# entn-at/exemplars_vc

Hardware: AMD Instinct MI355X
Metric: spectral frames/sec converted (100 NMF iters, N=4096 dict) (higher is better)
Workload: dtype f64

## Files before the change

exemplars_vc_amd/csrc/evc_fused_all.hip:

```cpp
#include "evc_fused_common.h"

namespace evc {

constexpr int AW = 4;
constexpr int AKT = 8;
constexpr int ATILES = AW * AKT;
constexpr int ATHREADS = 2 * AW * 64;
constexpr unsigned ALL_POLL_LIMIT = 1u << 17;
constexpr int ALL_STAGGER_PER_ITER = 11000;
constexpr int ALL_EXCH_PRIO = 3;
typedef unsigned all_u32x4 __attribute__((ext_vector_type(4)));
typedef long long all_i64x2 __attribute__((ext_vector_type(2)));

__device__ __forceinline__ bool all_polls_out(unsigned& polls, const int* coop_abort) {
    return ++polls > ALL_POLL_LIMIT ||
           ((polls & 63) == 0 && __hip_atomic_load(coop_abort, __ATOMIC_RELAXED, __HIP_MEMORY_SCOPE_AGENT) != 0);
}

constexpr long ALL_LDS_BUDGET = 160 * 1024 - 256;
__host__ __device__ constexpr int all_dict_row(int e) { return 4 * (((e >> 2) & 1) * 2 + (e >> 3)) + (e & 3); }
template <int MSTEPS, int C, bool KL>
struct AllShape {
    static constexpr int MT = MSTEPS > 4 ? 2 : 1;
    static constexpr int E = MT * 4 * 64;
    static constexpr int NE = MSTEPS * 64;
    static constexpr int RSTR = NE < 256 ? 256 : NE;
    static constexpr int STG = C > 0 ? 1 : (C == 0 ? NE : NE + ALL_MAX_MEMBERS - 1);
    static constexpr long REST = 8L * 2 * (AW * RSTR + 2 * E + (KL ? E : 1) + STG) + 3 * 4;
    static constexpr long dict_bytes(int pr) { return 8L * ATILES * 16 * pr; }
    static constexpr int PR_ALL = 4 * MSTEPS + 2;
    static constexpr int PR = KL ? 0
                              : REST + dict_bytes(PR_ALL) <= ALL_LDS_BUDGET       ? PR_ALL
                              : REST + dict_bytes(PR_ALL - 4) <= ALL_LDS_BUDGET   ? PR_ALL - 4
                                                                                  : 0;
    static constexpr bool LDS_DICT = C != 1 && PR > 0 && PR - 1 >= 4 * MSTEPS - 3;
};

#ifdef EVC_ALL_TIMING
#define EVC_STAMP(i)                                                                                             \
    do {                                                                                                         \
        if (a.dbg && tt0 == g - half && lane == 0 && w == 0)                                                     \
            a.dbg[(((long)blockIdx.x * 2 + half) * (2 * a.iters + 1) + step) * 4 + (i)] = __builtin_amdgcn_s_memtime(); \
    } while (0)
#else
#define EVC_STAMP(i)
#endif

template <int MSTEPS, int C, bool KL>
__global__ __launch_bounds__(ATHREADS, 2) void k_fused_all(FusedArgs a) {
    using S = AllShape<MSTEPS, C, KL>;
    constexpr int MT = S::MT;
    constexpr int E = S::E;
    constexpr int NE = S::NE;
    constexpr int RSTR = S::RSTR;
    constexpr int MSP = (MSTEPS + 1) & ~1;
    constexpr int PR = S::PR;
    constexpr int TPD = 16 * PR;
    __shared__ __attribute__((aligned(16))) double s_red[2][AW * RSTR];
    __shared__ __attribute__((aligned(16))) double s_v[2][E];
    __shared__ __attribute__((aligned(16))) double s_x[2][E];
    __shared__ __attribute__((aligned(16))) double s_r[2][KL ? E : 1];
    __shared__ double s_stage[2][S::STG];
    __shared__ double s_dict[S::LDS_DICT ? ATILES * TPD : 1];
    __shared__ unsigned s_hb[2];
    __shared__ int s_fail;
    const int tid = threadIdx.x, lane = tid & 63;
    const int w8 = __builtin_amdgcn_readfirstlane(tid >> 6);
    const int half = w8 >> 2, w = w8 & 3, th = tid & (AW * 64 - 1);
    const int CR = C > 0 ? C : a.coop_c;
    const int member = blockIdx.x % CR;
    const int g = 2 * (blockIdx.x / CR) + half;
    double* const red = s_red[half];
    double* const vL = s_v[half];
    double* const xL = s_x[half];
    double* const rL = s_r[half];
    double* const stage = s_stage[half];
    unsigned hb = 0;
    const double* __restrict__ A1p = a.A1p;
    const double* __restrict__ A2p = a.A2p;
    f64x2* __restrict__ Hp = a.Hp;
    const int NT = a.NT;
    const long tile0 = (long)member * ATILES + w;
    const unsigned ul = (unsigned)lane;
    long sw = 0;

    const __amdgpu_buffer_rsrc_t r1 = __builtin_amdgcn_make_buffer_rsrc(const_cast<double*>(A1p), 0, NT * (MSP * 512), 0x00020000);
    const __amdgpu_buffer_rsrc_t r2 = __builtin_amdgcn_make_buffer_rsrc(const_cast<double*>(A2p), 0, NT * (MT * 2048), 0x00020000);
    const __amdgpu_buffer_rsrc_t rx = __builtin_amdgcn_make_buffer_rsrc(a.coop_buf, 0, C > 1 ? 2 * a.groups * (C * 4096) : 0, 0x00020000);
#ifdef EVC_ALL_NOFRAG
    bool nofrag_go = false;
#endif
    const unsigned ul16 = ul * 16u;
    constexpr int BL = 16 * ((MSTEPS - 1) >> 2) + 4 * ((MSTEPS - 1) & 3);
    const int rowA = w * AKT * TPD + all_dict_row(4 * (lane & 3) + ((lane & 15) >> 2)) * PR;
    const int rowB = w * AKT * TPD + all_dict_row(4 * (lane >> 4)) * PR;
    const double* const dA = s_dict + rowA + (lane >> 4);
    const double* const dAL = s_dict + rowA + min(lane >> 4, a.M - BL);
    const double* const dB = s_dict + rowB + (lane & 15);
    const double* const dBL = s_dict + rowB + min(lane & 15, a.M - 16 * (MT - 1));
#define LDS_NO_PAIR() asm volatile("" ::: "memory")
    auto load_a1 = [&](double (&a1)[MSTEPS], int k, auto lds) {
        if constexpr (decltype(lds)::value) {
#pragma unroll
            for (int s = 0; s < MSTEPS; ++s) {
                a1[s] = (s == MSTEPS - 1 ? dAL : dA)[k * TPD + 16 * (s >> 2) + 4 * (s & 3)];
                LDS_NO_PAIR();
            }
            return;
        }
#ifdef EVC_ALL_NOFRAG
        if (nofrag_go) return;
#endif
        const int so = (int)(tile0 + sw + AW * k) * (MSP * 512);
#pragma unroll
        for (int s = 0; s < MSTEPS; s += 2) {
            if (s + 1 < MSTEPS) {
                const f64x2 v = __builtin_bit_cast(f64x2, __builtin_amdgcn_raw_buffer_load_b128(r1, ul16 + (s >> 1) * 1024, so, 0));
                a1[s] = v[0];
                a1[s + 1] = v[1];
            } else {
                a1[s] = __builtin_bit_cast(double, __builtin_amdgcn_raw_buffer_load_b64(r1, ul16 + (s >> 1) * 1024, so, 0));
            }
        }
    };
    auto load_a2 = [&](double (&a2)[MT][4], int k, auto lds) {
        if constexpr (decltype(lds)::value) {
#pragma unroll
            for (int u = 0; u < MT; ++u)
#pragma unroll
                for (int r = 0; r < 4; ++r) {
                    a2[u][r] = (u == MT - 1 ? dBL : dB)[k * TPD + r * PR + 16 * u];
                    LDS_NO_PAIR();
                }
            return;
        }
#ifdef EVC_ALL_NOFRAG
        if (nofrag_go) return;
#endif
        const int so = (int)(tile0 + sw + AW * k) * (MT * 2048);
#pragma unroll
        for (int u = 0; u < MT; ++u)
#pragma unroll
            for (int r = 0; r < 4; r += 2) {
                const f64x2 v = __builtin_bit_cast(f64x2, __builtin_amdgcn_raw_buffer_load_b128(r2, ul16 + (u * 2 + (r >> 1)) * 1024, so, 0));
                a2[u][r] = v[0];
                a2[u][r + 1] = v[1];
            }
    };

    const int mode = a.eps_mode;
    const double eps = a.eps;
    const double d0 = a.l1 + (mode == EVC_EPS_ADD ? a.eps : 0.0);
    const f64x4 dinit = {d0, d0, d0, d0};
    const unsigned lo = fast_lo(mode, eps);
    unsigned seq = 0;
    int rs_es = 1, rs_len = 0, rs_pub0 = 0, rs_pub1 = 0, rs_src0 = -1, rs_src1 = -1, rs_src2 = -1;
    if (C < 0) {
        rs_es = (NE + CR - 1) / CR;
        rs_len = NE - member * rs_es;
        rs_len = rs_len < 0 ? 0 : (rs_len > rs_es ? rs_es : rs_len);
        const int e0 = th, e1 = th + AW * 64;
        const int j0 = e0 / rs_es, j1 = (e1 < NE ? e1 : e0) / rs_es;
        rs_pub0 = (j0 * CR + member) * rs_es + (e0 - j0 * rs_es);
        rs_pub1 = (j1 * CR + member) * rs_es + ((e1 < NE ? e1 : e0) - j1 * rs_es);
        auto src = [&](int idx) {
            if (idx >= CR * rs_es) return -1;
            const int el = idx % rs_es;
            return el < rs_len ? member * CR * rs_es + idx : -1;
        };
        rs_src0 = src(th);
        rs_src1 = src(th + AW * 64);
        rs_src2 = src(th + 2 * AW * 64);
    }
    if (tid == 0) s_fail = 0;
    if (tid < 2) s_hb[tid] = 0;

    if (a.stagger_cycles > 0 && ((blockIdx.x / CR) & 1)) {
        const long long t0 = __builtin_amdgcn_s_memtime();
        while (__builtin_amdgcn_s_memtime() - t0 < a.stagger_cycles) __builtin_amdgcn_s_sleep(32);
    }

    auto run = [&](auto lds) __attribute__((always_inline)) {
    for (long tt0 = g - half; tt0 < a.TT; tt0 += a.groups) {
        const long tt = tt0 + half;
        bool valid;
        {
            const long t = 16 * tt + (lane & 15);
            int u = -1;
            if (tt < a.TT && t < a.T_) u = a.frame_utt[t];
            const bool live = tt < a.TT && ((t >= a.T_) || ((u >= 0) && (a.active[u] != 0)));
            const int v0 = __syncthreads_and(half == 0 ? live : true);
            const int v1 = __syncthreads_and(half == 1 ? live : true);
            valid = (half ? v1 : v0) != 0;
        }
        HTile h[AKT];
        f64x4 p[AKT];
        double a1[MSTEPS], a2[MT][4];
        if (valid && a.first && a.init_const) {
            auto h0_of = [&](int fr) {
                const long t = 16 * tt + fr;
                const int u = t < a.T_ ? a.frame_utt[t] : -1;
                return u >= 0 ? a.h0[u] : 0.0;
            };
            for (int e = th; e < E; e += AW * 64) {
                const int s = e >> 6, l = e & 63;
                const bool in = s < MSTEPS;
                xL[e] = in ? a.Xp[(tt * MSTEPS + s) * 64 + l] : 0.0;
                vL[e] = in ? a.rsum[bin_of(s, l >> 4)] * h0_of(l & 15) : 0.0;
                if (KL) rL[e] = xL[e] / (vL[e] < a.eps ? a.eps : vL[e]);
            }
            const double hv = h0_of(lane & 15);
#pragma unroll
            for (int k = 0; k < AKT; ++k) {
                const long n0 = 16 * (tile0 + AW * k) + 4 * (lane >> 4);
#pragma unroll
                for (int r = 0; r < 4; ++r) h[k][r] = n0 + r < a.N ? hv : 0.0;
            }
        } else if (valid) {
            for (int e = th; e < E; e += AW * 64) {
                const int s = e >> 6, l = e & 63;
                const bool in = s < MSTEPS;
                xL[e] = in ? a.Xp[(tt * MSTEPS + s) * 64 + l] : 0.0;
                vL[e] = in ? a.Vp[(tt * 8 + s) * 64 + l] : 0.0;
                if (KL) rL[e] = xL[e] / (vL[e] < a.eps ? a.eps : vL[e]);
            }
#pragma unroll
            for (int k = 0; k < AKT; ++k) {
                const f64x2* t = Hp + (tt * NT + tile0 + AW * k) * 128;
                const f64x2 h01 = t[ul], h23 = t[ul + 64];
                h[k][0] = h01[0]; h[k][1] = h01[1]; h[k][2] = h23[0]; h[k][3] = h23[1];
            }
        }
        __syncthreads();
        if (valid && !KL) {
            double x[MSTEPS];
#pragma unroll
            for (int s = 0; s < MSTEPS; ++s) x[s] = xL[s * 64 + lane];
            load_a1(a1, 0, lds);
#pragma unroll
            for (int k = 0; k < AKT; ++k) {
                f64x4 acc = {0, 0, 0, 0};
#pragma unroll
                for (int s = 0; s < MSTEPS; ++s) acc = Mma<double>::mma(a1[s], x[s], acc);
                if (!decltype(lds)::value || k + 1 < AKT) load_a1(a1, (k + 1) % AKT, lds);
                p[k] = acc;
            }
        }

        if (valid && KL) load_a1(a1, 0, lds);
        for (int step = 0; step <= 2 * a.iters; ++step) {
#ifdef EVC_ALL_NOFRAG
            nofrag_go = step > 2;
#endif
            const bool mine = C == 1 ? (step & 1) == 0 : (step & 1) == half;
            EVC_STAMP(0);
            if (valid && mine && step < 2 * a.iters) {
                asm volatile("" : "+s"(sw));
                double v[MSTEPS];
#pragma unroll
                for (int s = 0; s < MSTEPS; ++s) v[s] = KL ? rL[s * 64 + lane] : vL[s * 64 + lane];
                if constexpr (decltype(lds)::value) load_a1(a1, 0, lds);
                f64x4 vn[MT];
#pragma unroll
                for (int u = 0; u < MT; ++u) vn[u] = f64x4{0, 0, 0, 0};
#pragma unroll
                for (int k = 0; k < AKT; ++k) {
                    __builtin_amdgcn_sched_barrier(0);
                    load_a2(a2, k, lds);
                    f64x4 d = KL ? f64x4{0, 0, 0, 0} : dinit;
#pragma unroll
                    for (int s = 0; s < MSTEPS; ++s) d = Mma<double>::mma(a1[s], v[s], d);
                    if (!decltype(lds)::value || k + 1 < AKT)
                        load_a1(a1, (k + 1) % AKT, lds);
                    __builtin_amdgcn_sched_barrier(0);
                    if (KL) {
#pragma unroll
                        for (int r = 0; r < 4; ++r) h[k][r] *= d[r];
                    } else {
                        mu_tile_guarded(h[k], p[k], d, mode, eps, lo);
                    }
#pragma unroll
                    for (int u = 0; u < MT; ++u)
#pragma unroll
                        for (int r = 0; r < 4; ++r) vn[u] = Mma<double>::mma(a2[u][r], h[k][r], vn[u]);
                }
#pragma unroll
                for (int u = 0; u < MT; ++u)
#pragma unroll
                    for (int r = 0; r < 4; ++r)
                        if (u * 4 + r < MSTEPS) red[w * RSTR + (u * 4 + r) * 64 + lane] = vn[u][r];
            } else if (C > 1 && valid && !mine && step > 0) {
                __builtin_amdgcn_s_setprio(ALL_EXCH_PRIO);
                const bool act = th < NE / 2;
                const int ep = act ? 2 * th : 0;
                f64x2 sm = {0.0, 0.0};
                if (w * 64 < NE / 2) {
                    f64x2 pv[AW];
#pragma unroll
                    for (int ww = 0; ww < AW; ++ww) pv[ww] = *reinterpret_cast<const f64x2*>(red + ww * RSTR + ep);
                    static_assert(AW == 4, "the four partials are named one by one");
                    asm volatile("" : "+v"(pv[0]), "+v"(pv[1]), "+v"(pv[2]), "+v"(pv[3]));
#pragma unroll
                    for (int ww = 0; ww < AW; ++ww) sm += pv[ww];
                    const long long tag = (seq >> 1) & 1;
                    const long long m0 = (__double_as_longlong(sm[0]) & ~1LL) | tag;
                    const long long m1 = (__double_as_longlong(sm[1]) & ~1LL) | tag;
                    const int xo = __builtin_amdgcn_readfirstlane((int)(((seq & 1) * (unsigned)a.groups + (unsigned)g) * (unsigned)(C * 4096)));
                    if (act)
                        __builtin_amdgcn_raw_buffer_store_b128(__builtin_bit_cast(all_u32x4, all_i64x2{m0, m1}), rx, ep * 8,
                                                               xo + member * 4096, 16);
                    bool ok = true;
                    unsigned polls = 0;
                    {
                        const long long* sp = reinterpret_cast<const long long*>(a.coop_buf) +
                                              ((size_t)(seq & 1) * a.groups + g) * (size_t)(C * 512) +
                                              (lane < C ? lane : 0) * 512 + (NE - 1);
                        for (;;) {
                            const long long b = __hip_atomic_load(sp, __ATOMIC_RELAXED, __HIP_MEMORY_SCOPE_AGENT);
                            const bool ready = lane >= C || lane == member || (b & 1) == tag;
                            if (__all(ready)) break;
                            if (all_polls_out(polls, a.coop_abort)) {
                                ok = false;
                                break;
                            }
                            __builtin_amdgcn_s_sleep(2);
                        }
                    }
                    all_i64x2 b[C > 0 ? C : 1] = {};
                    polls = 0;
                    while (__builtin_expect(ok && act, 1)) {
                        asm volatile("" ::: "memory");
#pragma unroll
                        for (int m = 0; m < C; ++m)
                            if (m != member)
                                b[m] = __builtin_bit_cast(all_i64x2, __builtin_amdgcn_raw_buffer_load_b128(rx, ep * 8, xo + m * 4096, 16));
                        long long bad = 0;
#pragma unroll
                        for (int m = 0; m < C; ++m) {
                            b[m] = (m == member) ? all_i64x2{m0, m1} : b[m];
                            bad |= (b[m][0] ^ tag) | (b[m][1] ^ tag);
                        }
                        if ((bad & 1) == 0) break;
                        if (all_polls_out(polls, a.coop_abort)) {
                            ok = false;
                            break;
                        }
                        __builtin_amdgcn_s_sleep(2);
                    }
                    f64x2 v2 = {0.0, 0.0};
#pragma unroll
                    for (int m = 0; m < C; ++m) {
                        v2[0] += __longlong_as_double(b[m][0] & ~1LL);
                        v2[1] += __longlong_as_double(b[m][1] & ~1LL);
                    }
                    if (!ok) s_fail = 1;
                    if (act) {
                        *reinterpret_cast<f64x2*>(vL + ep) = v2;
                        if (KL) {
                            const f64x2 x2 = *reinterpret_cast<const f64x2*>(xL + ep);
                            *reinterpret_cast<f64x2*>(rL + ep) =
                                f64x2{x2[0] / (v2[0] < a.eps ? a.eps : v2[0]), x2[1] / (v2[1] < a.eps ? a.eps : v2[1])};
                        }
                    }
                }
                ++seq;
                __builtin_amdgcn_s_setprio(0);
            } else if (valid && !mine && step > 0) {
                const int e0 = C <= 0 ? th % NE : th, e1 = th + AW * 64;
                const bool has1 = e1 < NE;
                __builtin_amdgcn_s_setprio(ALL_EXCH_PRIO);
                double s0 = 0.0, s1 = 0.0;
#pragma unroll
                for (int ww = 0; ww < AW; ++ww) {
                    s0 += red[ww * RSTR + e0];
                    s1 += red[ww * RSTR + (has1 ? e1 : e0)];
                }
                if (C < 0) {
                    long long* xb1 = reinterpret_cast<long long*>(a.coop_buf) +
                                     ((size_t)(seq & 1) * a.groups + g) * (size_t)CR * ALL_RS_STRIDE;
                    long long* xb2 = reinterpret_cast<long long*>(a.coop_buf) + ALL_SLICE_OFFSET +
                                     ((size_t)(seq & 1) * a.groups + g) * 512;
                    const long long tag = (seq >> 1) & 1;
                    __hip_atomic_store(xb1 + rs_pub0, (__double_as_longlong(s0) & ~1LL) | tag, __ATOMIC_RELAXED,
                                       __HIP_MEMORY_SCOPE_AGENT);
                    if (has1)
                        __hip_atomic_store(xb1 + rs_pub1, (__double_as_longlong(s1) & ~1LL) | tag, __ATOMIC_RELAXED,
                                           __HIP_MEMORY_SCOPE_AGENT);
                    bool ok = true;
                    auto fetch3 = [&](const long long* p0, const long long* p1, const long long* p2, long long& b0,
                                      long long& b1, long long& b2) {
                        unsigned polls = 0;
                        for (;;) {
                            b0 = __hip_atomic_load(p0, __ATOMIC_RELAXED, __HIP_MEMORY_SCOPE_AGENT);
                            b1 = __hip_atomic_load(p1, __ATOMIC_RELAXED, __HIP_MEMORY_SCOPE_AGENT);
                            b2 = __hip_atomic_load(p2, __ATOMIC_RELAXED, __HIP_MEMORY_SCOPE_AGENT);
                            if (__all(!ok || (((b0 ^ tag) | (b1 ^ tag) | (b2 ^ tag)) & 1) == 0)) break;
                            if (all_polls_out(polls, a.coop_abort))
                                ok = false;
                            __builtin_amdgcn_s_sleep(1);
                        }
                    };
                    {
                        long long b0, b1, b2;
                        const long long* own = xb1 + rs_pub0;
                        fetch3(rs_src0 >= 0 ? xb1 + rs_src0 : own, rs_src1 >= 0 ? xb1 + rs_src1 : own,
                               rs_src2 >= 0 ? xb1 + rs_src2 : own, b0, b1, b2);
                        if (rs_src0 >= 0) stage[th] = __longlong_as_double(b0 & ~1LL);
                        if (rs_src1 >= 0) stage[th + AW * 64] = __longlong_as_double(b1 & ~1LL);
                        if (rs_src2 >= 0) stage[th + 2 * AW * 64] = __longlong_as_double(b2 & ~1LL);
                        hb += AW;
                        if (lane == 0)
                            __hip_atomic_fetch_add(&s_hb[half], 1u, __ATOMIC_RELEASE, __HIP_MEMORY_SCOPE_WORKGROUP);
                        while ((int)(__hip_atomic_load(&s_hb[half], __ATOMIC_ACQUIRE, __HIP_MEMORY_SCOPE_WORKGROUP) - hb) < 0)
                            __builtin_amdgcn_s_sleep(1);
                        const int q = th & 3;
                        for (int el = th >> 2; el < rs_len; el += AW * 16) {
                            double v = 0.0;
                            for (int m = q; m < CR; m += 4) v += stage[m * rs_es + el];
                            v += __shfl_xor(v, 1, 64);
                            v += __shfl_xor(v, 2, 64);
                            if (q == 0)
                                __hip_atomic_store(xb2 + member * rs_es + el, (__double_as_longlong(v) & ~1LL) | tag,
                                                   __ATOMIC_RELAXED, __HIP_MEMORY_SCOPE_AGENT);
                        }
                    }
                    long long g0, g1, g2;
                    fetch3(xb2 + e0, xb2 + (has1 ? e1 : e0), xb2 + e0, g0, g1, g2);
                    s0 = __longlong_as_double(g0 & ~1LL);
                    s1 = __longlong_as_double(g1 & ~1LL);
                    ++seq;
                    if (!ok) s_fail = 1;
                } else if (C == 0) {
                    const int ES = NE / CR;
                    long long* xb1 = reinterpret_cast<long long*>(a.coop_buf) +
                                     ((size_t)(seq & 1) * a.groups + g) * (size_t)CR * 512;
                    long long* xb2 = reinterpret_cast<long long*>(a.coop_buf) + ALL_SLICE_OFFSET +
                                     ((size_t)(seq & 1) * a.groups + g) * 512;
                    const long long tag = (seq >> 1) & 1;
                    {
                        const int j0 = e0 / ES, j1 = (has1 ? e1 : e0) / ES;
                        __hip_atomic_store(xb1 + ((size_t)j0 * CR + member) * ES + (e0 - j0 * ES),
                                           (__double_as_longlong(s0) & ~1LL) | tag, __ATOMIC_RELAXED,
                                           __HIP_MEMORY_SCOPE_AGENT);
                        if (has1)
                            __hip_atomic_store(xb1 + ((size_t)j1 * CR + member) * ES + (e1 - j1 * ES),
                                               (__double_as_longlong(s1) & ~1LL) | tag, __ATOMIC_RELAXED,
                                               __HIP_MEMORY_SCOPE_AGENT);
                    }
                    bool ok = true;
                    auto fetch2 = [&](const long long* p0, const long long* p1, long long& b0, long long& b1) {
                        unsigned polls = 0;
                        for (;;) {
                            b0 = __hip_atomic_load(p0, __ATOMIC_RELAXED, __HIP_MEMORY_SCOPE_AGENT);
                            b1 = __hip_atomic_load(p1, __ATOMIC_RELAXED, __HIP_MEMORY_SCOPE_AGENT);
                            if (__all(!ok || (((b0 ^ tag) | (b1 ^ tag)) & 1) == 0)) break;
                            if (all_polls_out(polls, a.coop_abort))
                                ok = false;
                            __builtin_amdgcn_s_sleep(1);
                        }
                    };
                    {
                        long long b0, b1;
                        const long long* mine_ = xb1 + (size_t)member * NE;
                        fetch2(mine_ + e0, mine_ + (has1 ? e1 : e0), b0, b1);
                        stage[e0] = __longlong_as_double(b0 & ~1LL);
                        if (has1) stage[e1] = __longlong_as_double(b1 & ~1LL);
                        hb += AW;
                        if (lane == 0)
                            __hip_atomic_fetch_add(&s_hb[half], 1u, __ATOMIC_RELEASE, __HIP_MEMORY_SCOPE_WORKGROUP);
                        while ((int)(__hip_atomic_load(&s_hb[half], __ATOMIC_ACQUIRE, __HIP_MEMORY_SCOPE_WORKGROUP) - hb) < 0)
                            __builtin_amdgcn_s_sleep(1);
                        if (th < 4 * ES) {
                            const int el = th >> 2, q = th & 3, per = CR >> 2;
                            double v = 0.0;
                            for (int i = 0; i < per; ++i) v += stage[(q * per + i) * ES + el];
                            v += __shfl_xor(v, 1, 64);
                            v += __shfl_xor(v, 2, 64);
                            if (q == 0)
                                __hip_atomic_store(xb2 + member * ES + el, (__double_as_longlong(v) & ~1LL) | tag,
                                                   __ATOMIC_RELAXED, __HIP_MEMORY_SCOPE_AGENT);
                        }
                    }
                    long long g0, g1;
                    fetch2(xb2 + e0, xb2 + (has1 ? e1 : e0), g0, g1);
                    s0 = __longlong_as_double(g0 & ~1LL);
                    s1 = __longlong_as_double(g1 & ~1LL);
                    ++seq;
                    if (!ok) s_fail = 1;
                }
                vL[e0] = s0;
                if (has1) vL[e1] = s1;
                if (KL) {
                    rL[e0] = xL[e0] / (s0 < a.eps ? a.eps : s0);
                    if (has1) rL[e1] = xL[e1] / (s1 < a.eps ? a.eps : s1);
                }
                __builtin_amdgcn_s_setprio(0);
            }
            EVC_STAMP(1);
            __syncthreads();
            EVC_STAMP(2);
            if (C != 1 && s_fail) {
                if (tid == 0) __hip_atomic_store(a.coop_abort, 1, __ATOMIC_RELAXED, __HIP_MEMORY_SCOPE_AGENT);
                return;
            }
        }

        auto y_tail = [&](auto ut) __attribute__((always_inline)) {
            constexpr int UT = decltype(ut)::value;
            f64x4 yn[UT];
#pragma unroll
            for (int u = 0; u < UT; ++u) yn[u] = f64x4{0, 0, 0, 0};
            if (valid) {
                const __amdgpu_buffer_rsrc_t rb = __builtin_amdgcn_make_buffer_rsrc(const_cast<double*>(a.Yb2p), 0, NT * (UT * 2048), 0x00020000);
#pragma unroll
                for (int k = 0; k < AKT; ++k) {
                    const int so = (int)(tile0 + AW * k) * (UT * 2048);
                    double b2[UT][4];
#pragma unroll
                    for (int u = 0; u < UT; ++u)
#pragma unroll
                        for (int r = 0; r < 4; r += 2) {
                            const f64x2 v = __builtin_bit_cast(f64x2, __builtin_amdgcn_raw_buffer_load_b128(rb, ul16 + (u * 2 + (r >> 1)) * 1024, so, 0));
                            b2[u][r] = v[0];
                            b2[u][r + 1] = v[1];
                        }
#pragma unroll
                    for (int u = 0; u < UT; ++u)
#pragma unroll
                        for (int r = 0; r < 4; ++r) yn[u] = Mma<double>::mma(b2[u][r], h[k][r], yn[u]);
                }
            }
#pragma unroll
            for (int u = 0; u < UT; ++u) {
                if (valid) {
#pragma unroll
                    for (int r = 0; r < 4; ++r) red[w * RSTR + r * 64 + lane] = yn[u][r];
                }
                __syncthreads();
                if (valid) {
                    double y = 0.0;
#pragma unroll
                    for (int ww = 0; ww < AW; ++ww) y += red[ww * RSTR + th];
                    a.Yslab[member * a.y_stride + (tt * 8 + 4 * u) * 64 + th] = y;
                }
                __syncthreads();
            }
        };
        if (a.Yslab) {
            if (MT > 1 && a.y_mt == 1) y_tail(std::integral_constant<int, 1>{});
            else y_tail(std::integral_constant<int, MT>{});
        }
        if (valid) {
            if (!a.skip_hp) {
#pragma unroll
                for (int k = 0; k < AKT; ++k) {
                    f64x2* t = Hp + (tt * NT + tile0 + AW * k) * 128;
                    t[ul] = f64x2{h[k][0], h[k][1]};
                    t[ul + 64] = f64x2{h[k][2], h[k][3]};
                }
            }
            if (a.Hx) {
                const long t = 16 * tt + (lane & 15);
                if (t < a.T_ && a.hx_wide) {
#pragma unroll
                    for (int k = 0; k < AKT; ++k) {
                        const long n0 = 16 * (tile0 + AW * k) + 4 * (lane >> 4);
                        double* const row = a.Hx + t * a.ldhx + n0;
#pragma unroll
                        for (int r = 0; r < 4; r += 2) {
                            if (n0 + r + 1 < a.N) *reinterpret_cast<f64x2*>(row + r) = f64x2{h[k][r], h[k][r + 1]};
                            else if (n0 + r < a.N) row[r] = h[k][r];
                        }
                    }
                } else if (t < a.T_) {
#pragma unroll
                    for (int k = 0; k < AKT; ++k) {
                        const long n0 = 16 * (tile0 + AW * k) + 4 * (lane >> 4);
#pragma unroll
                        for (int r = 0; r < 4; ++r)
                            if (n0 + r < a.N) {
                                if (a.hx_frame_major) a.Hx[t * a.ldhx + n0 + r] = h[k][r];
                                else a.Hx[(n0 + r) * a.ldhx + t] = h[k][r];
                            }
                    }
                }
            }
            if (member == 0) {
                for (int e = th; e < NE; e += AW * 64) a.Vp[(tt * 8 + (e >> 6)) * 64 + (e & 63)] = vL[e];
                if (a.write_err && w == 0) {
                    double e = 0.0;
#pragma unroll
                    for (int s = 0; s < MSTEPS; ++s) {
                        const double x = xL[s * 64 + lane], vv = vL[s * 64 + lane];
                        e += KL ? kl_terms(x, vv, a.eps) : (x - vv) * (x - vv);
                    }
                    e += __shfl_xor(e, 16, 64);
                    e += __shfl_xor(e, 32, 64);
                    const long t = 16 * tt + lane;
                    if (lane < 16 && t < a.T_) a.err2[t] = e;
                }
            }
        }
        __syncthreads();
    }
    };

    if constexpr (S::LDS_DICT) {
        if (a.M > 0 && a.M < PR) {
            for (int x = tid; x < ATILES * TPD; x += ATHREADS) {
                const int slot = x / TPD, e = all_dict_row((x / PR) % 16), b = x % PR;
                const long j = (long)member * ATILES + slot / AKT + AW * (slot % AKT);
                const int q = e >> 2, r = e & 3;
                s_dict[x] = b < a.M ? A2p[((j * MT + (b >> 4)) * 2 + (r >> 1)) * 128 + (16 * q + (b & 15)) * 2 + (r & 1)] : 0.0;
            }
            __syncthreads();
            run(std::true_type{});
            return;
        }
    }
    run(std::false_type{});
}

template <int MSTEPS, int C, bool KL>
static hipError_t launch_all(FusedArgs a, int n_cus, hipStream_t s) {
    int occ = 0;
    hipError_t e = hipOccupancyMaxActiveBlocksPerMultiprocessor(&occ, k_fused_all<MSTEPS, C, KL>, ATHREADS, 0);
    if (e != hipSuccess) return e;
    if (occ < 1) return hipErrorInvalidValue;
    long resident = n_cus;
    if (2 * resident > ALL_MAX_WGS) resident = ALL_MAX_WGS / 2;
    const int cr = C > 0 ? C : a.coop_c;
    if (C == 0 && (cr < 8 || cr > 64 || (cr & (cr - 1)))) return hipErrorInvalidValue;
    if (C < 0 && (cr < 2 || cr > ALL_MAX_MEMBERS)) return hipErrorInvalidValue;
    int pairs = (int)(resident / cr);
    const int want = (a.TT + 1) / 2;
    if (pairs > want) pairs = want;
    if (pairs < 1) return hipErrorInvalidValue;
    a.groups = 2 * pairs;
    a.stagger_cycles = (a.iters > 0 && a.iters <= 25 && a.TT >= 4L * a.groups && pairs >= 2) ? (long long)a.iters * ALL_STAGGER_PER_ITER : 0;
    if (C > 1 && (reinterpret_cast<uintptr_t>(a.coop_buf) & 15)) return hipErrorInvalidValue;
    if (C != 1) {
        e = hipMemsetAsync(a.coop_buf, 0xFF, sizeof(double) * 2 * (size_t)a.groups * cr * (C < 0 ? ALL_RS_STRIDE : 512), s);
        if (e != hipSuccess) return e;
    }
    if (C <= 0) {
        if (2L * a.groups * 512 > ALL_SLICE_ELEMS) return hipErrorInvalidValue;
        e = hipMemsetAsync(a.coop_buf + ALL_SLICE_OFFSET, 0xFF, sizeof(double) * 2 * (size_t)a.groups * 512, s);
        if (e != hipSuccess) return e;
    }
    hipLaunchKernelGGL((k_fused_all<MSTEPS, C, KL>), dim3((unsigned)(pairs * cr)), dim3(ATHREADS), 0, s, a);
    return hipGetLastError();
}

template <int MSTEPS, bool KL>
static hipError_t pick_c(const FusedArgs& a, int n_cus, hipStream_t s) {
    switch (a.NT / ATILES) {
        case 1: return launch_all<MSTEPS, 1, KL>(a, n_cus, s);
        case 2: return launch_all<MSTEPS, 2, KL>(a, n_cus, s);
        case 4: return launch_all<MSTEPS, 4, KL>(a, n_cus, s);
        case 8:
            if constexpr (AllShape<MSTEPS, 8, KL>::LDS_DICT)
                if (a.M > 0 && a.M < AllShape<MSTEPS, 8, KL>::PR) return launch_all<MSTEPS, 8, KL>(a, n_cus, s);
            return launch_all<MSTEPS, 0, KL>(a, n_cus, s);
        case 16:
        case 32:
        case 64: return launch_all<MSTEPS, 0, KL>(a, n_cus, s);
        default: return launch_all<MSTEPS, -1, KL>(a, n_cus, s);
    }
}

int fused_all_members(int NT, int N, int eps_mode, int exact_div, int loss) {
    if (eps_mode == EVC_EPS_NONE || exact_div || (loss != EVC_LOSS_FROBENIUS && loss != EVC_LOSS_KL)) return 0;
    if (NT % ATILES) return 0;
    const int c = NT / ATILES;
    if (loss == EVC_LOSS_KL && c >= 2 && c < 16) return 0;
    return (c >= 1 && c <= ALL_MAX_MEMBERS) ? c : 0;
}

hipError_t fused_all_launch(int msteps, const FusedArgs& a, int n_cus, hipStream_t s) {
    if (a.NT % ATILES || !a.coop_buf || !a.coop_abort) return hipErrorInvalidValue;
    switch (msteps) {
        case 1: return a.loss == EVC_LOSS_KL ? pick_c<1, true>(a, n_cus, s) : pick_c<1, false>(a, n_cus, s);
        case 2: return a.loss == EVC_LOSS_KL ? pick_c<2, true>(a, n_cus, s) : pick_c<2, false>(a, n_cus, s);
        case 3: return a.loss == EVC_LOSS_KL ? pick_c<3, true>(a, n_cus, s) : pick_c<3, false>(a, n_cus, s);
        case 4: return a.loss == EVC_LOSS_KL ? pick_c<4, true>(a, n_cus, s) : pick_c<4, false>(a, n_cus, s);
        case 5: return a.loss == EVC_LOSS_KL ? pick_c<5, true>(a, n_cus, s) : pick_c<5, false>(a, n_cus, s);
        case 6: return a.loss == EVC_LOSS_KL ? pick_c<6, true>(a, n_cus, s) : pick_c<6, false>(a, n_cus, s);
        case 7: return a.loss == EVC_LOSS_KL ? pick_c<7, true>(a, n_cus, s) : pick_c<7, false>(a, n_cus, s);
        case 8: return a.loss == EVC_LOSS_KL ? pick_c<8, true>(a, n_cus, s) : pick_c<8, false>(a, n_cus, s);
        default: return hipErrorInvalidValue;
    }
}

}
```

Baseline: 1.130 million.

## Prefetch next-step operands before the block barrier and double-buffer fail flags

When the dictionary lives in LDS and blocks cooperate, each half now loads its next-step v/r operands and first dictionary fragment right after finishing the current step. It first meets the other waves of its half at a per-half rendezvous, so the LDS loads overlap the __syncthreads wait instead of starting after it. The shared fail flag is split into two parity slots and read one step later, so the abort check no longer depends on a value written in the same step; a final check after the loop covers both slots. This adds extra intra-half spin synchronisation and holds the operand registers across the barrier, which may raise register pressure. Timing instrumentation is also extended to stamp every tile.

New measurement: 1.140 million, median of 6. Within noise of the previous version (+0.8%).

```diff
diff --git a/exemplars_vc_amd/csrc/evc_fused_all.hip b/exemplars_vc_amd/csrc/evc_fused_all.hip
--- a/exemplars_vc_amd/csrc/evc_fused_all.hip
+++ b/exemplars_vc_amd/csrc/evc_fused_all.hip
@@ -26,7 +26,7 @@
     static constexpr int NE = MSTEPS * 64;
     static constexpr int RSTR = NE < 256 ? 256 : NE;
     static constexpr int STG = C > 0 ? 1 : (C == 0 ? NE : NE + ALL_MAX_MEMBERS - 1);
-    static constexpr long REST = 8L * 2 * (AW * RSTR + 2 * E + (KL ? E : 1) + STG) + 3 * 4;
+    static constexpr long REST = 8L * 2 * (AW * RSTR + 2 * E + (KL ? E : 1) + STG) + 4 * 4;
     static constexpr long dict_bytes(int pr) { return 8L * ATILES * 16 * pr; }
     static constexpr int PR_ALL = 4 * MSTEPS + 2;
     static constexpr int PR = KL ? 0
@@ -37,13 +37,22 @@
 };
 
 #ifdef EVC_ALL_TIMING
+#define EVC_STAMP_ROW()                                                                                          \
+    const long dbg_row = (((long)blockIdx.x * 2 + half) * ((a.TT + a.groups - 1) / a.groups) + (tt0 - (g - half)) / a.groups) * \
+                         (2 * a.iters + 1)
 #define EVC_STAMP(i)                                                                                             \
     do {                                                                                                         \
-        if (a.dbg && tt0 == g - half && lane == 0 && w == 0)                                                     \
-            a.dbg[(((long)blockIdx.x * 2 + half) * (2 * a.iters + 1) + step) * 4 + (i)] = __builtin_amdgcn_s_memtime(); \
+        if (a.dbg && lane == 0 && w == 0) a.dbg[(dbg_row + step) * 4 + (i)] = __builtin_amdgcn_s_memtime();        \
+    } while (0)
+#define EVC_STAMP_OPERANDS()                                                                                     \
+    do {                                                                                                         \
+        asm volatile("s_waitcnt lgkmcnt(0)" ::: "memory");                                                       \
+        EVC_STAMP(3);                                                                                            \
     } while (0)
 #else
+#define EVC_STAMP_ROW()
 #define EVC_STAMP(i)
+#define EVC_STAMP_OPERANDS()
 #endif
 
 template <int MSTEPS, int C, bool KL>
@@ -63,7 +72,7 @@
     __shared__ double s_stage[2][S::STG];
     __shared__ double s_dict[S::LDS_DICT ? ATILES * TPD : 1];
     __shared__ unsigned s_hb[2];
-    __shared__ int s_fail;
+    __shared__ int s_fail[2];
     const int tid = threadIdx.x, lane = tid & 63;
     const int w8 = __builtin_amdgcn_readfirstlane(tid >> 6);
     const int half = w8 >> 2, w = w8 & 3, th = tid & (AW * 64 - 1);
@@ -172,7 +181,7 @@
         rs_src1 = src(th + AW * 64);
         rs_src2 = src(th + 2 * AW * 64);
     }
-    if (tid == 0) s_fail = 0;
+    if (tid < 2) s_fail[tid] = 0;
     if (tid < 2) s_hb[tid] = 0;
 
     if (a.stagger_cycles > 0 && ((blockIdx.x / CR) & 1)) {
@@ -183,6 +192,7 @@
     auto run = [&](auto lds) __attribute__((always_inline)) {
     for (long tt0 = g - half; tt0 < a.TT; tt0 += a.groups) {
         const long tt = tt0 + half;
+        EVC_STAMP_ROW();
         bool valid;
         {
             const long t = 16 * tt + (lane & 15);
@@ -248,18 +258,37 @@
         }
 
         if (valid && KL) load_a1(a1, 0, lds);
+        double v[MSTEPS];
+        constexpr bool PRE = decltype(lds)::value && C != 1;
+        auto next_operands = [&]() __attribute__((always_inline)) {
+#pragma unroll
+            for (int s = 0; s < MSTEPS; ++s) v[s] = KL ? rL[s * 64 + lane] : vL[s * 64 + lane];
+            load_a1(a1, 0, lds);
+        };
+        auto half_rendezvous = [&]() __attribute__((always_inline)) {
+            hb += AW;
+            if (lane == 0) __hip_atomic_fetch_add(&s_hb[half], 1u, __ATOMIC_RELEASE, __HIP_MEMORY_SCOPE_WORKGROUP);
+            while ((int)(__hip_atomic_load(&s_hb[half], __ATOMIC_ACQUIRE, __HIP_MEMORY_SCOPE_WORKGROUP) - hb) < 0)
+                __builtin_amdgcn_s_sleep(1);
+        };
+        if constexpr (PRE) {
+            if (valid) next_operands();
+        }
         for (int step = 0; step <= 2 * a.iters; ++step) {
 #ifdef EVC_ALL_NOFRAG
             nofrag_go = step > 2;
 #endif
             const bool mine = C == 1 ? (step & 1) == 0 : (step & 1) == half;
             EVC_STAMP(0);
+            const int failed = C != 1 ? s_fail[(step & 1) ^ 1] : 0;
             if (valid && mine && step < 2 * a.iters) {
                 asm volatile("" : "+s"(sw));
-                double v[MSTEPS];
-#pragma unroll
-                for (int s = 0; s < MSTEPS; ++s) v[s] = KL ? rL[s * 64 + lane] : vL[s * 64 + lane];
-                if constexpr (decltype(lds)::value) load_a1(a1, 0, lds);
+                if constexpr (!PRE) {
+#pragma unroll
+                    for (int s = 0; s < MSTEPS; ++s) v[s] = KL ? rL[s * 64 + lane] : vL[s * 64 + lane];
+                    if constexpr (decltype(lds)::value) load_a1(a1, 0, lds);
+                }
+                EVC_STAMP_OPERANDS();
                 f64x4 vn[MT];
 #pragma unroll
                 for (int u = 0; u < MT; ++u) vn[u] = f64x4{0, 0, 0, 0};
@@ -353,7 +382,7 @@
                         v2[0] += __longlong_as_double(b[m][0] & ~1LL);
                         v2[1] += __longlong_as_double(b[m][1] & ~1LL);
                     }
-                    if (!ok) s_fail = 1;
+                    if (!ok) s_fail[step & 1] = 1;
                     if (act) {
                         *reinterpret_cast<f64x2*>(vL + ep) = v2;
                         if (KL) {
@@ -364,6 +393,10 @@
                     }
                 }
                 ++seq;
+                if constexpr (PRE) {
+                    half_rendezvous();
+                    next_operands();
+                }
                 __builtin_amdgcn_s_setprio(0);
             } else if (valid && !mine && step > 0) {
                 const int e0 = C <= 0 ? th % NE : th, e1 = th + AW * 64;
@@ -429,7 +462,7 @@
                     s0 = __longlong_as_double(g0 & ~1LL);
                     s1 = __longlong_as_double(g1 & ~1LL);
                     ++seq;
-                    if (!ok) s_fail = 1;
+                    if (!ok) s_fail[step & 1] = 1;
                 } else if (C == 0) {
                     const int ES = NE / CR;
                     long long* xb1 = reinterpret_cast<long long*>(a.coop_buf) +
@@ -486,7 +519,7 @@
                     s0 = __longlong_as_double(g0 & ~1LL);
                     s1 = __longlong_as_double(g1 & ~1LL);
                     ++seq;
-                    if (!ok) s_fail = 1;
+                    if (!ok) s_fail[step & 1] = 1;
                 }
                 vL[e0] = s0;
                 if (has1) vL[e1] = s1;
@@ -494,15 +527,23 @@
                     rL[e0] = xL[e0] / (s0 < a.eps ? a.eps : s0);
                     if (has1) rL[e1] = xL[e1] / (s1 < a.eps ? a.eps : s1);
                 }
+                if constexpr (PRE) {
+                    half_rendezvous();
+                    next_operands();
+                }
                 __builtin_amdgcn_s_setprio(0);
             }
             EVC_STAMP(1);
             __syncthreads();
             EVC_STAMP(2);
-            if (C != 1 && s_fail) {
+            if (C != 1 && failed) {
                 if (tid == 0) __hip_atomic_store(a.coop_abort, 1, __ATOMIC_RELAXED, __HIP_MEMORY_SCOPE_AGENT);
                 return;
             }
+        }
+        if (C != 1 && (s_fail[0] | s_fail[1])) {
+            if (tid == 0) __hip_atomic_store(a.coop_abort, 1, __ATOMIC_RELAXED, __HIP_MEMORY_SCOPE_AGENT);
+            return;
         }
 
         auto y_tail = [&](auto ut) __attribute__((always_inline)) {
```
